# simonsysu/tfs

Measured on AMD Instinct MI355X. Metric: GiB/s CRC32 verify, device-resident 64 KiB files; 1/2/4/8 MI355X, higher is better.
Workload: dtype u8

## Files before the change

### tfs_amd/csrc/tfs_crc_abi.cpp

```cpp
#include <emmintrin.h>
#include <hip/hip_runtime.h>

#include <algorithm>
#include <atomic>
#include <chrono>
#include <condition_variable>
#include <cstdarg>
#include <cstdio>
#include <cstdlib>
#include <cstring>
#include <map>
#include <memory>
#include <mutex>
#include <shared_mutex>
#include <string>
#include <vector>

#include "../../include/tfs_crc.h"
#include "../../include/tfs_crc_testing.h"
#include "../../include/tfs_read.h"
#include "../../include/tfs_receive.h"
#include "../../include/tfs_replicate.h"
#include "../../include/tfs_write.h"
#include "crc_math.h"
#include "pin_registry.h"
#include "mirror_plan.h"
#include "read_reply_plan.h"
#include "receive_plan.h"
#include "replicate_plan.h"
#include "tfs_crc_device.h"

namespace tfscrc {
hipError_t launch_crc_files(int mode, const uint8_t* base, const Desc* desc, uint32_t n, const Tables* tg,
                            uint32_t* out_crc, uint8_t* out_ok, uint32_t* n_bad, uint32_t* sched, hipStream_t stream,
                            int variant, uint32_t vseed, uint32_t* done_flag, uint32_t seq, unsigned cap,
                            const SplitArgs* split);
hipError_t launch_packet_parse(const uint8_t* base, const PacketDesc* pd, uint32_t n, int mode, Desc* desc,
                               int32_t* pre, hipStream_t stream);
hipError_t launch_packet_files(uint8_t* base, const PacketDesc* pd, uint32_t n, int mode, const Tables* tg,
                               uint32_t* crc, int32_t* status, uint32_t* n_bad, uint32_t* sched, hipStream_t stream,
                               unsigned cap);
hipError_t launch_packet_finish(uint8_t* base, const PacketDesc* pd, const Desc* desc, uint32_t n, int mode,
                                const int32_t* pre, const uint8_t* ok, uint32_t* crc, int32_t* status,
                                uint32_t* n_bad, hipStream_t stream);
hipError_t launch_packet_write(const uint8_t* base, const PacketDesc* pd, uint32_t n, const Tables* tg, uint32_t* crc,
                               int32_t* status, uint32_t* n_bad, WritePart* parts, uint32_t* sched,
                               hipStream_t stream, unsigned cap);
hipError_t launch_packet_write_parse(const uint8_t* base, const PacketDesc* pd, uint32_t n, Desc* desc, int32_t* pre,
                                     Desc* hdesc, WritePart* parts, hipStream_t stream);
hipError_t launch_packet_data_fold(const Tables* tg, uint32_t n, const int32_t* status, const uint32_t* crc,
                                   const uint32_t* pcrc, WritePart* parts, hipStream_t stream);
hipError_t launch_crc_shift(const Tables* tg, const uint32_t* crc, const uint32_t* nbytes, uint32_t n, uint32_t* out,
                            hipStream_t stream);
hipError_t launch_block_verify_pipe(const uint8_t* image, uint64_t image_len, const RawMeta* metas,
                                    const CompactJob* jobs, uint32_t n, const Tables* tg, uint32_t* out_crc,
                                    int32_t* out_status, uint32_t* n_bad, uint32_t* sched, hipStream_t stream,
                                    int variant, unsigned cap);
hipError_t launch_compact_fused(const uint8_t* src, uint64_t src_len, const RawMeta* metas, const int32_t* flags,
                                const int64_t* dest_off, uint32_t n, uint8_t* dst, const Tables* tg, uint32_t* out_crc,
                                int32_t* out_status, uint32_t* n_bad, uint32_t* sched, hipStream_t stream,
                                int variant, unsigned cap);
hipError_t launch_compact_jobs(const uint8_t* src, uint64_t src_len, const CompactJob* jobs, uint32_t n, uint8_t* dst,
                               const Tables* tg, uint32_t* out_crc, int32_t* out_status, uint32_t* n_bad,
                               uint32_t* sched, hipStream_t stream, int variant, unsigned cap, const CSegArgs* seg);
hipError_t launch_read_reply(const uint8_t* src, uint64_t src_len, const ReadUnit* units, uint32_t n, uint8_t* out,
                             const Tables* tg, ReadResult* results, uint32_t* n_bad, uint32_t* sched,
                             hipStream_t stream, unsigned cap);
hipError_t launch_replicate(const uint8_t* src, uint64_t src_len, const RepUnit* units, uint32_t nu,
                            const RepFrame* frames, uint32_t nf, uint8_t* out, const Tables* tg, uint32_t* ucrc,
                            uint8_t* cap_bytes, uint32_t* racc, uint32_t* fcrc, uint32_t* sched, hipStream_t stream,
                            unsigned cap);
hipError_t launch_replicate_finish(const RepRec* recs, uint32_t n, const uint8_t* cap_bytes, const uint32_t* racc,
                                   uint32_t* out_crc, int32_t* out_status, hipStream_t stream);
hipError_t launch_receive(const uint8_t* src, const RecvFrame* frames, uint32_t nf, uint32_t nu, uint8_t* image,
                          const Tables* tg, uint32_t* ucrc, uint32_t block_id, uint32_t* words, tfs_receive_part* parts,
                          uint32_t* n_bad, uint32_t* sched, hipStream_t stream, unsigned cap);
hipError_t launch_receive_finish(const RecvRec* recs, uint32_t n, const uint8_t* image, const uint32_t* words,
                                 uint32_t* out_crc, int32_t* out_status, hipStream_t stream);
hipError_t launch_mirror(const uint8_t* src, uint64_t src_len, const MirJob* jobs, uint32_t nj, const MirFrame* frames,
                         uint32_t nf, const MirUnit* units, uint32_t nu, const uint8_t* prefix, uint8_t* out,
                         const Tables* tg, uint32_t* ucrc, uint8_t* cap_bytes, int32_t* jstat, MirResult* results,
                         uint32_t* n_bad, uint32_t* sched, hipStream_t stream, unsigned cap);
hipError_t launch_synth_fill(uint64_t* dst, uint64_t nwords, uint64_t seed, uint64_t first_word, hipStream_t stream);
hipError_t launch_write_headers(uint8_t* image, const uint64_t* rec_off, const uint32_t* len, const uint32_t* crc,
                                uint64_t first_id, uint32_t n, hipStream_t stream);
hipError_t launch_write_packet_headers(uint8_t* base, const uint64_t* rec_off, const uint32_t* len, uint32_t n,
                                       int32_t pcode, int32_t version, uint64_t first_id, hipStream_t stream);
#ifdef TFS_CRC_MEASURE
hipError_t set_res_fence(uint32_t v);
hipError_t launch_membench(int pattern, const uint8_t* base, const Desc* desc, uint32_t n, uint64_t nbytes,
                           uint32_t* out, unsigned grid, hipStream_t stream);
#endif
hipError_t launch_resident(const Tables* tg, const ResHost* hs, uint32_t* left, uint32_t* dstate, unsigned grid,
                           uint32_t idle_ticks,
                           uint32_t life_ticks, uint32_t gen, hipStream_t stream, uint64_t* trace);
}

namespace tfscrc {

namespace {
struct PinRange {
  uintptr_t end;
  uintptr_t dev;
};
std::shared_mutex g_pin_mu;
std::map<uintptr_t, PinRange> g_pins;
}

void pin_register(void* host, size_t bytes, void* dev) {
  if (!host || !dev) return;
  const uintptr_t h = reinterpret_cast<uintptr_t>(host);
  std::unique_lock<std::shared_mutex> g(g_pin_mu);
  g_pins[h] = PinRange{h + (bytes ? bytes : 1), reinterpret_cast<uintptr_t>(dev)};
}

void pin_unregister(void* host) {
  if (!host) return;
  std::unique_lock<std::shared_mutex> g(g_pin_mu);
  g_pins.erase(reinterpret_cast<uintptr_t>(host));
}

bool pin_lookup(const void* p, void** dev) {
  const uintptr_t a = reinterpret_cast<uintptr_t>(p);
  std::shared_lock<std::shared_mutex> g(g_pin_mu);
  auto it = g_pins.upper_bound(a);
  if (it == g_pins.begin()) return false;
  --it;
  if (a >= it->second.end) return false;
  if (dev) *dev = reinterpret_cast<void*>(it->second.dev + (a - it->first));
  return true;
}

}

static_assert(sizeof(tfs_crc_desc) == 16 && sizeof(tfs_crc_vdesc) == 16, "descriptor ABI");
static_assert(sizeof(tfs_raw_meta) == sizeof(tfscrc::RawMeta), "RawMeta ABI");
static_assert(sizeof(tfs_file_info) == 36, "FileInfo ABI");
static_assert(sizeof(tfs_crc_stats) == 64, "stats ABI");
static_assert(sizeof(tfs_packet_desc) == sizeof(tfscrc::PacketDesc), "packet descriptor ABI");
static_assert(sizeof(tfs_write_part) == sizeof(tfscrc::WritePart) && sizeof(tfs_write_part) == 16, "write part ABI");
static_assert(sizeof(tfs_compact_job) == sizeof(tfscrc::CompactJob) && sizeof(tfs_compact_job) == 40, "compact job ABI");
static_assert(sizeof(tfs_read_job) == 48 && sizeof(tfs_read_result) == 16, "read reply ABI");
static_assert(sizeof(tfs_replicate_cfg) == 32, "replicate cfg ABI");
static_assert(sizeof(tfs_receive_cfg) == 16 && sizeof(tfs_receive_desc) == 24 && sizeof(tfs_receive_part) == 16,
              "receive ABI");
static_assert(sizeof(tfs_mirror_cfg) == 16 && sizeof(tfs_mirror_job) == 64 && sizeof(tfs_mirror_result) == 16,
              "mirror ABI");

namespace {

using namespace tfscrc;

struct DevBuf {
  void* p = nullptr;
  size_t cap = 0;
  hipError_t reserve(size_t bytes) {
    if (bytes <= cap) return hipSuccess;
    if (p) (void)hipFree(p);
    p = nullptr;
    cap = 0;
    size_t want = std::max<size_t>(bytes, 4096);
// ... 2782 lines not shown
  if (n == 0) return TFS_SUCCESS;
  HIP_TRY(ctx, hipSetDevice(ctx->device));
  hipStream_t st = ctx->stream;
  const size_t pbytes = size_t(n) * sizeof(tfs_receive_part);
  HIP_TRY(ctx, s->d_parts.reserve(pbytes + 4u));
  HIP_TRY(ctx, s->h_parts.reserve(pbytes + 4u));
  tfs_receive_part* d_parts = static_cast<tfs_receive_part*>(s->d_parts.p);
  uint32_t* d_bad = reinterpret_cast<uint32_t*>(static_cast<uint8_t*>(s->d_parts.p) + pbytes);
  HIP_TRY(ctx, hipMemsetAsync(d_bad, 0, 4u, st));
  void* zbase = nullptr;
  const bool zc = is_pinned_host(base) && host_dev_ptr(base, &zbase);
  (void)hipGetLastError();
  if (zc) {
    if (const int rc = recv_enqueue(s, st, static_cast<const uint8_t*>(zbase), descs, n, d_parts, d_bad)) return rc;
  } else {
    const uint64_t piece = std::max<uint64_t>(ctx->read_piece.load(std::memory_order_relaxed), 1u);
    const uint8_t* b8 = static_cast<const uint8_t*>(base);
    std::vector<tfs_receive_desc> pd;
    for (uint32_t j0 = 0; j0 < n;) {
      uint64_t lo = UINT64_MAX, hi = 0;
      uint32_t j1 = j0;
      pd.clear();
      for (; j1 < n; ++j1) {
        tfs_receive_desc d = descs[j1];
        d.avail = kRecvOverhead + uint32_t(d.data_len);
        const uint64_t nlo = std::min(lo, d.frame_off), nhi = std::max(hi, d.frame_off + d.avail);
        if (j1 > j0 && nhi - nlo > piece) break;
        lo = nlo, hi = nhi;
        pd.push_back(d);
      }
      const uint64_t span = hi - lo, sa = lo & 15u;
      HIP_TRY(ctx, s->h_stage.reserve(span + 32u));
      HIP_TRY(ctx, s->d_stage.reserve(span + 32u));
      memcpy(static_cast<uint8_t*>(s->h_stage.p) + sa, b8 + lo, span);
      HIP_TRY(ctx, hipMemcpyAsync(static_cast<uint8_t*>(s->d_stage.p) + sa, static_cast<uint8_t*>(s->h_stage.p) + sa, span,
                                  hipMemcpyHostToDevice, st));
      for (auto& d : pd) d.frame_off -= lo;
      if (const int rc = recv_enqueue(s, st, static_cast<const uint8_t*>(s->d_stage.p) + sa, pd.data(), j1 - j0,
                                      d_parts + j0, d_bad))
        return rc;
      HIP_TRY(ctx, hipStreamSynchronize(st));
      j0 = j1;
    }
  }
  HIP_TRY(ctx, hipMemcpyAsync(s->h_parts.p, s->d_parts.p, pbytes + 4u, hipMemcpyDeviceToHost, st));
  HIP_TRY(ctx, hipStreamSynchronize(st));
  memcpy(parts, s->h_parts.p, pbytes);
  if (n_bad) {
    uint32_t bad = 0;
    memcpy(&bad, static_cast<const uint8_t*>(s->h_parts.p) + pbytes, 4u);
    *n_bad += bad;
  }
  s->stream = st, s->stream_set = true;
  s->cursor = end;
  return TFS_SUCCESS;
}

int tfs_receive_finish(tfs_receive* s, const tfs_raw_meta* metas, uint32_t n, uint32_t* out_crc, int32_t* out_status,
                       uint32_t* n_bad, int32_t* out_total) {
  if (!s) return TFS_EXIT_PARAMETER_ERROR;
  tfs_crc_ctx* ctx = s->ctx;
  if (s->finished) return set_err(ctx, TFS_EXIT_PARAMETER_ERROR, "receive finish: called twice");
  if (n && !metas) return set_err(ctx, TFS_EXIT_PARAMETER_ERROR, "receive finish: %u records and no metas", n);
  HIP_TRY(ctx, hipSetDevice(ctx->device));
  s->finished = true;
  hipStream_t st = s->stream_set ? s->stream : ctx->stream;
  if (!s->waited) {
    if (st != ctx->stream) HIP_TRY(ctx, hipStreamWaitEvent(st, s->ready, 0));
    s->waited = true;
  }
  const uint32_t* hr = nullptr;
  if (n) {
    s->recs.resize(n);
    s->res.resize(size_t(n) * 2u);
    for (uint32_t i = 0; i < n; ++i) s->recs[i] = recv_make_rec(metas[i], s->cursor);
    const size_t rbytes = size_t(n) * sizeof(RecvRec);
    uint8_t* d_fin = s->fin();
    if (n > kRecvFinRecs) {
      HIP_TRY(ctx, s->d_fin.reserve(rbytes + size_t(n) * 8u));
      d_fin = static_cast<uint8_t*>(s->d_fin.p);
    }
    uint32_t* d_crc = reinterpret_cast<uint32_t*>(d_fin + rbytes);
    HIP_TRY(ctx, hipMemcpyAsync(d_fin, s->recs.data(), rbytes, hipMemcpyHostToDevice, st));
    HIP_TRY(ctx, launch_receive_finish(reinterpret_cast<const RecvRec*>(d_fin), n, s->d_image, s->words(), d_crc,
                                       reinterpret_cast<int32_t*>(d_crc + n), st));
    HIP_TRY(ctx, hipMemcpyAsync(s->res.data(), d_crc, size_t(n) * 8u, hipMemcpyDeviceToHost, st));
    hr = s->res.data();
  }
  HIP_TRY(ctx, hipStreamSynchronize(st));
  uint32_t bad = 0;
  for (uint32_t i = 0; i < n; ++i) {
    const int32_t status = int32_t(hr[n + i]);
    if (out_crc) out_crc[i] = hr[i];
    if (out_status) out_status[i] = status;
    bad += status != TFS_SUCCESS ? 1u : 0u;
  }
  if (n_bad) *n_bad += bad;
  if (out_total) *out_total = int32_t(s->cursor);
  return TFS_SUCCESS;
}

int tfs_receive_free(tfs_receive* s) {
  if (!s) return TFS_EXIT_PARAMETER_ERROR;
  (void)hipSetDevice(s->ctx->device);
  if (s->stream_set) (void)hipStreamSynchronize(s->stream);
  if (!s->waited && s->ready) (void)hipEventSynchronize(s->ready);
  s->release();
  delete s;
  return TFS_SUCCESS;
}


extern "C++" {
namespace {

int mir_call_checks(tfs_crc_ctx* ctx, const tfs_mirror_cfg* cfg, const void* src, uint64_t src_len,
                    const tfs_mirror_job* jobs, uint32_t n, const uint64_t* ds, uint32_t ds_n, const void* out,
                    uint64_t out_cap, const void* results, std::vector<int32_t>* pre) {
  if (!cfg || !out || !results || (n && !jobs) || (ds_n && !ds) || (src_len && !src)) return TFS_EXIT_PARAMETER_ERROR;
  if (!mir_cfg_ok(*cfg))
    return set_err(ctx, TFS_EXIT_PARAMETER_ERROR, "mirror: first_len %d, frame_len %d, reserved %d are refused",
                   cfg->first_len, cfg->frame_len, int(cfg->reserved));
  pre->resize(n);
  for (uint32_t i = 0; i < n; ++i) (*pre)[i] = mir_pre_status(*cfg, jobs[i], ds_n, src_len, out_cap);
  if (mir_spans_overlap(*cfg, jobs, pre->data(), n))
    return set_err(ctx, TFS_EXIT_PARAMETER_ERROR, "mirror: the spans of two jobs overlap");
  return TFS_SUCCESS;
}

int mir_enqueue(tfs_crc_ctx* ctx, hipStream_t st, const uint8_t* d_src, uint64_t src_len, const tfs_mirror_cfg& cfg,
                const tfs_mirror_job* jobs, const int32_t* pre, uint32_t n, const uint64_t* ds, uint8_t* d_out,
                tfs_mirror_result* d_results, uint32_t* d_n_bad) {
  std::lock_guard<std::mutex> g(ctx->mir_mu);
  MirPlan& p = ctx->mir_plan;
  if (!make_mirror_plan(cfg, jobs, pre, n, ds, &p))
    return set_err(ctx, TFS_EXIT_PARAMETER_ERROR, "mirror: more than 2^31 frames or units in one call");
  const uint32_t nf = uint32_t(p.frames.size()), nu = uint32_t(p.units.size());
  const size_t o_frames = up16(size_t(n) * sizeof(MirJob)), o_units = o_frames + size_t(nf) * sizeof(MirFrame);
  const size_t o_prefix = o_units + size_t(nu) * sizeof(MirUnit), plan_bytes = up16(o_prefix + p.prefix.size());
  const size_t o_ucrc = plan_bytes, o_cap = o_ucrc + up16(size_t(nu) * 4u);
  const size_t o_jstat = o_cap + up16(size_t(n) * kFileInfoSize), total = o_jstat + size_t(n) * 4u;
  ReadPlanSlot& rp = ctx->mir_plans[ctx->mir_plan_next++ % kReadPlanRing];
  if (rp.done) HIP_TRY(ctx, hipEventSynchronize(rp.done));
  HIP_TRY(ctx, rp.h.reserve(plan_bytes));
  HIP_TRY(ctx, rp.d.reserve(total));
  uint8_t* h8 = static_cast<uint8_t*>(rp.h.p);
  uint8_t* d8 = static_cast<uint8_t*>(rp.d.p);
  memcpy(h8, p.jobs.data(), size_t(n) * sizeof(MirJob));
  if (nf) memcpy(h8 + o_frames, p.frames.data(), size_t(nf) * sizeof(MirFrame));
  if (nu) memcpy(h8 + o_units, p.units.data(), size_t(nu) * sizeof(MirUnit));
  if (!p.prefix.empty()) memcpy(h8 + o_prefix, p.prefix.data(), p.prefix.size());
  HIP_TRY(ctx, hipMemcpyAsync(d8, h8, plan_bytes, hipMemcpyHostToDevice, st));
  SCHED_LAUNCH(ctx, st, "mirror",
               launch_mirror(d_src, src_len, reinterpret_cast<const MirJob*>(d8), n,
                             reinterpret_cast<const MirFrame*>(d8 + o_frames), nf,
                             reinterpret_cast<const MirUnit*>(d8 + o_units), nu, d8 + o_prefix, d_out, ctx->d_tables,
                             reinterpret_cast<uint32_t*>(d8 + o_ucrc), d8 + o_cap,
                             reinterpret_cast<int32_t*>(d8 + o_jstat), d_results, d_n_bad, sched, st,
                             throughput_cap(ctx)));
  if (!rp.done) HIP_TRY(ctx, hipEventCreateWithFlags(&rp.done, hipEventDisableTiming));
  HIP_TRY(ctx, hipEventRecord(rp.done, st));
  return TFS_SUCCESS;
}

}
}

// ... 538 lines not shown
```

### tfs_amd/csrc/tfs_crc_kernels.hip

```cpp
#include <hip/hip_runtime.h>
#include <stdint.h>

#include <type_traits>

#include "mirror_plan.h"
#include "read_reply_plan.h"
#include "receive_plan.h"
#include "replicate_plan.h"
#include "tfs_crc_device.h"

namespace tfscrc {

typedef const __attribute__((address_space(1))) uint32_t* gu32p;
typedef unsigned int u32x4 __attribute__((ext_vector_type(4)));
typedef const __attribute__((address_space(1))) u32x4* gu128p;
typedef const __attribute__((address_space(1))) uint8_t* gu8p;
__device__ __forceinline__ uint32_t ld32(uintptr_t a) { return *reinterpret_cast<gu32p>(a); }
__device__ __forceinline__ uint4 ld128(uintptr_t a) {
  const u32x4 v = *reinterpret_cast<gu128p>(a);
  return make_uint4(v.x, v.y, v.z, v.w);
}
template <bool NT>
__device__ __forceinline__ uint4 ld128s(uintptr_t a) {
  if (NT) {
// ... 2046 lines not shown
  const uint32_t g = off / kRecvG + (f - u0);
  const uint64_t gs = uint64_t(g) * kRecvG, fe = uint64_t(off) + len;
  const uint64_t start = gs > off ? gs : uint64_t(off);
  const uint64_t end = gs + kRecvG < fe ? gs + kRecvG : fe;
  RepUnit u{};
  u.soff = soff + kRecvHead + (start - off);
  u.doff = start;
  u.plen = uint32_t(end - start);
  src_end = recv_uni(frames[lo].src_end);
  return u;
}

__global__ void __launch_bounds__(kBlock, 4) receive_kernel(const uint8_t* __restrict__ src,
                                                            const RecvFrame* __restrict__ frames_in, uint32_t nf,
                                                            uint32_t n, uint8_t* __restrict__ image,
                                                            const Tables* __restrict__ tg, uint32_t* __restrict__ ucrc,
                                                            uint32_t* sched) {
  __shared__ uint32_t lds_tables[LdsLayout<kLY>::bytes / 4];
  __shared__ uint32_t lds_frames[kRecvLdsFrames * sizeof(RecvFrame) / 4];
  if (nf <= kRecvLdsFrames) {
    const uint32_t* f32 = reinterpret_cast<const uint32_t*>(frames_in);
    for (uint32_t k = threadIdx.x; k < nf * uint32_t(sizeof(RecvFrame) / 4); k += kBlock) lds_frames[k] = f32[k];
  }
  load_tables<kRun, kPAR, kLY>(lds_tables, tg);
  __syncthreads();
  const RecvFrame* frames = nf <= kRecvLdsFrames ? reinterpret_cast<const RecvFrame*>(lds_frames) : frames_in;
  const int lane = threadIdx.x & (kWave - 1);
  const LaneBase lb = lane_base_for<kLY>(lane);
  const uint32_t wpb = kBlock / kWave;
  const uintptr_t junk = reinterpret_cast<uintptr_t>(tg->slice);
  FileCursor<kIL, 1, 0, kCompactHS> fc;
  fc.init(sched, n, blockIdx.x & 7u, gridDim.x * wpb,
          blockIdx.x * wpb + __builtin_amdgcn_readfirstlane(threadIdx.x / kWave));
  fc.start(lane);
  do {
    uint32_t f = __builtin_amdgcn_readfirstlane(fc.take(lane));
    if (f >= n) break;
    uint32_t fn = __builtin_amdgcn_readfirstlane(fc.take(lane));
    uint64_t cur_end = 0, nxt_end = 0;
    RepUnit cur = recv_unit(frames, nf, f, cur_end);
    CState st = issue_rep(cur, src, cur_end, image, lane, junk);
    uint4 buf[kPF][kRun / 16];
    load_ring<kRun, kPF, false>(st.g, lane, buf, junk);
    RepUnit nxt = fn < n ? recv_unit(frames, nf, fn, nxt_end) : RepUnit{};
    for (;;) {
      const bool more = fn < n;
      const RepUnit ncur = nxt;
      uint32_t c = st.g.nstripes ? lane_chain<kRun, kPF, false, kLY, true, true, 1>(lds_tables, lb, st.g, st.h, buf,
                                                                                    lane, junk, st.delta, true)
                                 : 0u;
      CState ns = st;
      uint32_t fnn = n;
      if (more) {
        ns = issue_rep(ncur, src, nxt_end, image, lane, junk);
        load_ring<kRun, kPF, false>(ns.g, lane, buf, junk);
        fnn = __builtin_amdgcn_readfirstlane(fc.take(lane));
        if (fnn < n) nxt = recv_unit(frames, nf, fnn, nxt_end);
      }
      if (st.g.nstripes) {
        if (lane == 0) {
          const uint32_t ntw = uint32_t((st.g.end & ~uintptr_t(3)) - st.g.B16) / 4u;
          for (uint32_t i = 0; i < 3u; ++i)
            if (i < ntw) st32u(st.g.B16 + 4u * i + st.delta, st.h.tw[i]);
          const uintptr_t B = st.g.end & ~uintptr_t(3);
          for (uint32_t i = 0; i < 3u; ++i)
            if (B + i < st.g.end) *reinterpret_cast<uint8_t*>(B + i + st.delta) = uint8_t(st.h.tb[i]);
        }
      } else {
        copy_unaligned(src + cur.soff, image + cur.doff, cur.plen, lane);
      }
      c = finish_file<kRun, kLY>(lds_tables, lb, st.g, st.h, c, lane);
      if (lane == 0) ucrc[f] = c;
      if (!more) break;
      f = fn;
      fn = fnn;
      cur = ncur;
      st = ns;
    }
  } while (false);
  if (lane == 0) launch_exit(sched, gridDim.x * wpb, nullptr, 0u);
}

__device__ const RecvPowTab kRecvPow = recv_pow_tab();
__device__ __forceinline__ uint32_t recv_pow(uint32_t d) {
  uint32_t r = 0x80000000u;
  for (uint32_t k = 0; d; ++k, d >>= 1)
    if (d & 1u) r = gf_mul(r, kRecvPow.p[k]);
  return r;
}

__device__ __forceinline__ uint32_t recv_byte_crc(uint32_t b) {
#pragma unroll
  for (int k = 0; k < 8; ++k) b = (b >> 1) ^ ((b & 1u) ? kPoly : 0u);
  return b;
}

__device__ __forceinline__ uint32_t recv_wave_xor(uint32_t x) {
#pragma unroll
  for (int m = kWave / 2; m >= 1; m >>= 1) x ^= __shfl_xor(x, m, kWave);
  return x;
}

__device__ __forceinline__ uint32_t recv_dword(uint32_t hb, uint32_t k) {
  return __shfl(hb, int(4u * k), kWave) | __shfl(hb, int(4u * k + 1u), kWave) << 8 |
         __shfl(hb, int(4u * k + 2u), kWave) << 16 | __shfl(hb, int(4u * k + 3u), kWave) << 24;
}

__global__ void __launch_bounds__(kWave) receive_fold_kernel(const uint8_t* __restrict__ src,
                                                             const RecvFrame* __restrict__ frames,
                                                             const uint32_t* __restrict__ ucrc, uint32_t block_id,
                                                             uint32_t* words, tfs_receive_part* __restrict__ parts,
                                                             uint32_t* n_bad) {
  const RecvFrame fr = frames[blockIdx.x];
  const uint32_t lane = threadIdx.x;
  const uint8_t* frame = src + fr.soff;
  uint32_t hb = 0u;
  if (lane < kRecvHead) hb = frame[lane];
  else if (lane < kRecvOverhead) hb = frame[uint64_t(fr.len) + lane];
  const uint32_t h_flag = recv_dword(hb, 0), h_body = recv_dword(hb, 1), h_tv = recv_dword(hb, 2);
  const uint32_t h_crc = recv_dword(hb, 5), i_block = recv_dword(hb, 6), i_off = recv_dword(hb, 9);
  const uint32_t i_len = recv_dword(hb, 10), flag = recv_dword(hb, 14);
  const bool in_h = lane >= 24u && lane < kRecvHead, in_f = lane >= kRecvHead && lane < kRecvOverhead;
  const uint32_t bc = (in_h || in_f) ? gf_mul(recv_byte_crc(hb), recv_pow(in_h ? 55u - lane : 59u - lane)) : 0u;
  const uint32_t ch = recv_wave_xor(in_h ? bc : 0u), cf = recv_wave_xor(in_f ? bc : 0u);
  uint32_t x = 0u;
  const uint32_t g0 = fr.off / kRecvG, fe = fr.off + fr.len;
  const uint32_t nb = fr.nu ? fr.nu - 1u : 0u;
  const uint32_t per = (nb + kWave - 1u) / kWave;
  const uint32_t k0 = lane * per, k1 = k0 + per < nb ? k0 + per : nb;
  uint32_t acc = 0u;
  for (uint32_t k = k0; k < k1; ++k) {
    const uint32_t c = ucrc[fr.u0 + k];
    acc = gf_mul(acc, kRecvPow.p[kRecvLgG]) ^ c;
    if ((g0 + k) * kRecvG >= fr.off) words[g0 + k] = c;
    else atomicXor(&words[g0 + k], c);
  }
  if (k0 < k1) x = gf_mul(acc, recv_pow(fe - (g0 + k1) * kRecvG));
  if (lane == kWave - 1 && fr.nu) {
    const uint32_t c = ucrc[fr.u0 + nb];
    const uint32_t gs = (g0 + nb) * kRecvG;
    x ^= c;
    if (gs >= fr.off && fe == gs + kRecvG) words[g0 + nb] = c;
    else atomicXor(&words[g0 + nb], gf_mul(c, recv_pow(gs + kRecvG - fe)));
  }
  x = recv_wave_xor(x);
  if (lane == 0) {
    const uint32_t chs = ch ^ gf_mul(kPacketFlagV1, kRecvPow.p[5]);
    const uint32_t body = gf_mul(chs, recv_pow(fr.len + 4u)) ^ gf_mul(x, kRecvPow.p[2]) ^ cf;
    const int32_t version = int16_t(uint16_t(h_tv >> 16));
    int32_t status = kSuccess;
    if (h_flag != kPacketFlagV1) status = TFS_ERROR;
    else if (h_body != kRecvInfo + fr.len) status = TFS_ERROR;
    else if ((h_tv & 0xffffu) != uint32_t(TFS_RECEIVE_PCODE)) status = TFS_ERROR;
    else if (i_block != block_id) status = TFS_ERROR;
    else if (i_off != fr.off || i_len != fr.len) status = TFS_ERROR;
    else if (version >= 1 && h_crc != body) status = kExitCheckCrcError;
    parts[blockIdx.x] = tfs_receive_part{status, version >= 1 ? body : 0u, int32_t(flag), 0u};
    if (status != kSuccess && n_bad) atomicAdd(n_bad, 1u);
  }
}

__device__ __forceinline__ uint32_t recv_edge(const uint8_t* __restrict__ image, uint32_t lo, uint32_t hi, uint32_t b,
                                              uint32_t lane) {
  constexpr uint32_t kPer = kRecvG / kWave;
  if (hi - lo <= lane * kPer) return 0u;
  const uint32_t e = hi - lane * kPer;
  const uint32_t s = e - lo > kPer ? e - kPer : lo;
  uint32_t c = 0u;
  for (uint32_t i = s; i < e; ++i) {
    c ^= image[i];
#pragma unroll
    for (int k = 0; k < 8; ++k) c = (c >> 1) ^ ((c & 1u) ? kPoly : 0u);
  }
  return gf_mul(c, recv_pow(b - e));
}

__global__ void __launch_bounds__(kWave) receive_finish_kernel(const RecvRec* __restrict__ recs, uint32_t n,
                                                                const uint8_t* __restrict__ image,
                                                                const uint32_t* __restrict__ words,
                                                                uint32_t* __restrict__ out_crc,
                                                                int32_t* __restrict__ out_status) {
  const uint32_t i = blockIdx.x;
  if (i >= n) return;
  const uint32_t lane = threadIdx.x;
  const RecvRec r = recs[i];
  if (r.pre != kSuccess) {
    if (lane == 0) out_crc[i] = 0u, out_status[i] = r.pre;
    return;
  }
  const uint32_t hb = lane < kRecvInfo ? uint32_t(image[uint64_t(uint32_t(r.offset)) + lane]) : 0u;
  const uint64_t id = uint64_t(recv_dword(hb, 0)) | uint64_t(recv_dword(hb, 1)) << 32;
  const uint32_t fi_size = recv_dword(hb, 3), fi_crc = recv_dword(hb, 8);
  uint32_t x = recv_edge(image, r.a, r.he, r.b, lane) ^ recv_edge(image, r.tb, r.b, r.b, lane);
  if (lane < r.ng) {
    const uint32_t mstep = kRecvPow.p[kRecvLgG + 6u];
    uint32_t acc = 0u, first = 0u;
    for (uint32_t k = lane % kWave; k < r.ng; k += kWave) first = k;
    for (uint32_t k = first;; k -= kWave) {
      acc = gf_mul(acc, mstep) ^ words[r.g0 + r.ng - 1u - k];
      if (k < kWave) break;
    }
    x ^= gf_mul(acc, recv_pow(r.b - (r.g0 + r.ng - lane) * kRecvG));
  }
  x = recv_wave_xor(x);
  if (lane == 0) {
    int32_t status = kSuccess;
    if (id != r.file_id) status = kExitFileInfoError;
    else if (int32_t(fi_size) != r.size) status = kExitSyncFileError;
    else if (x != fi_crc) status = kExitCheckCrcError;
    out_crc[i] = x;
    out_status[i] = status;
  }
}

__device__ __forceinline__ CState issue_mir(const MirUnit& u, const uint8_t* src, uint64_t src_len, uint8_t* out,
                                            int lane, uintptr_t junk) {
  CRec r;
  r.soff = u.soff - kFileInfoSize;
  r.doff = u.doff - kFileInfoSize;
  r.fid = 0;
  r.size = 0, r.flag = 0, r.new_off = 0;
  r.pre = kSuccess;
  r.plen = u.plen;
  r.kind = 1u;
  r.edge = 0u;
  CState s = issue_crec<true>(r, src, src_len, out, lane, junk);
  s.hb = (u.job & kMirStart) && lane < kFileInfoSize ? uint32_t(src[r.soff + uint32_t(lane)]) : 0u;
  return s;
}

__global__ void __launch_bounds__(kBlock, 4) mirror_kernel(const uint8_t* __restrict__ src, uint64_t src_len,
                                                           const MirUnit* __restrict__ units, uint32_t n,
                                                           uint8_t* __restrict__ out, const Tables* __restrict__ tg,
                                                           uint32_t* __restrict__ ucrc, uint8_t* __restrict__ cap,
                                                           uint32_t* sched) {
  __shared__ uint32_t lds_tables[LdsLayout<kLY>::bytes / 4];
  load_tables<kRun, kPAR, kLY>(lds_tables, tg);
  const int lane = threadIdx.x & (kWave - 1);
  const LaneBase lb = lane_base_for<kLY>(lane);
  const uint32_t wpb = kBlock / kWave;
  const uintptr_t junk = reinterpret_cast<uintptr_t>(tg->slice);
  FileCursor<kIL, 1, 0, kCompactHS> fc;
  fc.init(sched, n, blockIdx.x & 7u, gridDim.x * wpb,
          blockIdx.x * wpb + __builtin_amdgcn_readfirstlane(threadIdx.x / kWave));
  fc.start(lane);
  do {
    uint32_t f = fc.take(lane);
    if (f >= n) break;
    uint32_t fn = fc.take(lane);
    MirUnit cur = units[f];
    CState st = issue_mir(cur, src, src_len, out, lane, junk);
    uint4 buf[kPF][kRun / 16];
    load_ring<kRun, kPF, false>(st.g, lane, buf, junk);
    MirUnit nxt = fn < n ? units[fn] : MirUnit{};
    for (;;) {
      const bool more = fn < n;
      const MirUnit ncur = nxt;
      uint32_t c = st.g.nstripes ? lane_chain<kRun, kPF, false, kLY, true, true, 1>(lds_tables, lb, st.g, st.h, buf,
                                                                                    lane, junk, st.delta, true)
                                 : 0u;
      CState ns = st;
      uint32_t fnn = n;
      if (more) {
        ns = issue_mir(ncur, src, src_len, out, lane, junk);
        load_ring<kRun, kPF, false>(ns.g, lane, buf, junk);
        fnn = fc.take(lane);
        if (fnn < n) nxt = units[fnn];
      }
      if ((cur.job & kMirStart) && lane < kFileInfoSize)
        cap[uint64_t(cur.job & ~kMirStart) * kFileInfoSize + uint32_t(lane)] = uint8_t(st.hb);
      if (st.g.nstripes) {
        if (lane == 0) {
          const uint32_t ntw = uint32_t((st.g.end & ~uintptr_t(3)) - st.g.B16) / 4u;
          for (uint32_t i = 0; i < 3u; ++i)
            if (i < ntw) st32u(st.g.B16 + 4u * i + st.delta, st.h.tw[i]);
          const uintptr_t B = st.g.end & ~uintptr_t(3);
          for (uint32_t i = 0; i < 3u; ++i)
            if (B + i < st.g.end) *reinterpret_cast<uint8_t*>(B + i + st.delta) = uint8_t(st.h.tb[i]);
        }
      } else {
        copy_unaligned(src + cur.soff, out + cur.doff, cur.plen, lane);
      }
      c = finish_file<kRun, kLY>(lds_tables, lb, st.g, st.h, c, lane);
      if (lane == 0) ucrc[f] = c;
      if (!more) break;
// ... 729 lines not shown
  else if (variant == 96) TFS_CJ(12, 2, 2, 3, kCompactDiag);
  else if (variant == 97) TFS_CJ(16, 1, 2, kPF, kCompactDiag);
  else if (variant == 98) TFS_CJ(10, 2, 2, kPF, kCompactDiag);
  else if (variant == 99) TFS_CJ(16, 2, 2, 3, kCompactDiag);
  else if (variant == 120) TFS_CJR(16, 1, 2, kPF, kCompactDiag, true);
  else if (variant == 121) TFS_CJR(8, 1, 2, 8, kCompactDiag, true);
  else
#endif
    TFS_CJ(16, 1, kLY, kPF, kCompactDiag);
#undef TFS_CJ
#undef TFS_CJR
  (void)variant;
  return hipGetLastError();
}

hipError_t launch_block_verify_pipe(const uint8_t* image, uint64_t image_len, const RawMeta* metas,
                                    const CompactJob* jobs, uint32_t n, const Tables* tg, uint32_t* out_crc,
                                    int32_t* out_status, uint32_t* n_bad, uint32_t* sched, hipStream_t stream,
                                    int variant, unsigned cap) {
  if (n == 0) return hipSuccess;
  if (!sched) return hipErrorInvalidValue;
  const dim3 grid(grid_for(n, cap));
#define TFS_BV(WIDE_, CF_, TS_)                                                                                     \
  hipLaunchKernelGGL((compact_pipe_kernel<WIDE_, true, kCompactDiag, kPF, CF_, TS_>), grid, dim3(kBlock), 0, stream, \
                     image, image_len, metas, nullptr, nullptr, jobs, n, nullptr, tg, out_crc, out_status, n_bad, sched, \
                     CSegArgs{nullptr, 0u, 0u})
#ifdef TFS_CRC_MEASURE
  if (variant == 50 && jobs) TFS_BV(true, 1, 0);
  else if (variant == 50) TFS_BV(false, 1, 0);
  else
#endif
  if (jobs) TFS_BV(true, kCF, kTS);
  else TFS_BV(false, kCF, kTS);
#undef TFS_BV
  (void)variant;
  return hipGetLastError();
}

hipError_t launch_read_reply(const uint8_t* src, uint64_t src_len, const ReadUnit* units, uint32_t n, uint8_t* out,
                             const Tables* tg, ReadResult* results, uint32_t* n_bad, uint32_t* sched,
                             hipStream_t stream, unsigned cap) {
  if (n == 0) return hipSuccess;
  if (!sched) return hipErrorInvalidValue;
  hipLaunchKernelGGL(read_reply_kernel, dim3(grid_for(n, cap)), dim3(kBlock), 0, stream, src, src_len, units, n, out,
                     tg, results, n_bad, sched);
  return hipGetLastError();
}

hipError_t launch_replicate(const uint8_t* src, uint64_t src_len, const RepUnit* units, uint32_t nu,
                            const RepFrame* frames, uint32_t nf, uint8_t* out, const Tables* tg, uint32_t* ucrc,
                            uint8_t* cap_bytes, uint32_t* racc, uint32_t* fcrc, uint32_t* sched, hipStream_t stream,
                            unsigned cap) {
  if (nf == 0) return hipSuccess;
  if (nu) {
    if (!sched) return hipErrorInvalidValue;
    hipLaunchKernelGGL(replicate_kernel, dim3(grid_for(nu, cap)), dim3(kBlock), 0, stream, src, src_len, units, nu, out,
                       tg, ucrc, cap_bytes, sched);
    const hipError_t e = hipGetLastError();
    if (e != hipSuccess) return e;
  }
  hipLaunchKernelGGL(replicate_fold_kernel, dim3(nf), dim3(kWave), 0, stream, frames, units, ucrc, out, racc, fcrc);
  return hipGetLastError();
}

hipError_t launch_replicate_finish(const RepRec* recs, uint32_t n, const uint8_t* cap_bytes, const uint32_t* racc,
                                   uint32_t* out_crc, int32_t* out_status, hipStream_t stream) {
  if (n == 0) return hipSuccess;
  hipLaunchKernelGGL(replicate_finish_kernel, dim3((n + 255u) / 256u), dim3(256), 0, stream, recs, n, cap_bytes, racc,
                     out_crc, out_status);
  return hipGetLastError();
}

hipError_t launch_receive(const uint8_t* src, const RecvFrame* frames, uint32_t nf, uint32_t nu, uint8_t* image,
                          const Tables* tg, uint32_t* ucrc, uint32_t block_id, uint32_t* words, tfs_receive_part* parts,
                          uint32_t* n_bad, uint32_t* sched, hipStream_t stream, unsigned cap) {
  if (nf == 0) return hipSuccess;
  if (nu) {
    if (!sched) return hipErrorInvalidValue;
    hipLaunchKernelGGL(receive_kernel, dim3(grid_for(nu, cap)), dim3(kBlock), 0, stream, src, frames, nf, nu, image, tg,
                       ucrc, sched);
    const hipError_t e = hipGetLastError();
    if (e != hipSuccess) return e;
  }
  hipLaunchKernelGGL(receive_fold_kernel, dim3(nf), dim3(kWave), 0, stream, src, frames, ucrc, block_id, words, parts,
                     n_bad);
  return hipGetLastError();
}

hipError_t launch_receive_finish(const RecvRec* recs, uint32_t n, const uint8_t* image, const uint32_t* words,
                                 uint32_t* out_crc, int32_t* out_status, hipStream_t stream) {
  if (n == 0) return hipSuccess;
  hipLaunchKernelGGL(receive_finish_kernel, dim3(n), dim3(kWave), 0, stream, recs, n, image, words,
                     out_crc, out_status);
  return hipGetLastError();
}

hipError_t launch_mirror(const uint8_t* src, uint64_t src_len, const MirJob* jobs, uint32_t nj, const MirFrame* frames,
                         uint32_t nf, const MirUnit* units, uint32_t nu, const uint8_t* prefix, uint8_t* out,
                         const Tables* tg, uint32_t* ucrc, uint8_t* cap_bytes, int32_t* jstat, MirResult* results,
                         uint32_t* n_bad, uint32_t* sched, hipStream_t stream, unsigned cap) {
  if (nj == 0) return hipSuccess;
  if (nu) {
    if (!sched) return hipErrorInvalidValue;
    hipLaunchKernelGGL(mirror_kernel, dim3(grid_for(nu, cap)), dim3(kBlock), 0, stream, src, src_len, units, nu, out, tg,
                       ucrc, cap_bytes, sched);
    const hipError_t e = hipGetLastError();
    if (e != hipSuccess) return e;
  }
  hipLaunchKernelGGL(mirror_job_fold_kernel, dim3(nj), dim3(kWave), 0, stream, jobs, units, ucrc, cap_bytes, results,
                     jstat, n_bad);
  const hipError_t e = hipGetLastError();
  if (e != hipSuccess || nf == 0) return e;
  hipLaunchKernelGGL(mirror_frame_fold_kernel, dim3(nf), dim3(kWave), 0, stream, frames, jobs, units, ucrc, prefix, jstat,
                     out);
  return hipGetLastError();
}

hipError_t launch_synth_fill(uint64_t* dst, uint64_t nwords, uint64_t seed, uint64_t first_word, hipStream_t stream) {
  if (nwords == 0) return hipSuccess;
  uint64_t g = (nwords + 255) / 256;
  if (g > 65536) g = 65536;
  hipLaunchKernelGGL(synth_fill_kernel, dim3(unsigned(g)), dim3(256), 0, stream, dst, nwords, seed, first_word);
  return hipGetLastError();
}

#ifdef TFS_CRC_MEASURE
template <int PF, int SK, int HOLE = 0>
__global__ void __launch_bounds__(kBlock) membench_copy_chunk_kernel(const uint8_t* __restrict__ src,
                                                                     uint8_t* __restrict__ dst, uint64_t nbytes,
                                                                     uint64_t ch) {
  const int lane = threadIdx.x & (kWave - 1);
  const uint64_t wave = uint64_t(blockIdx.x) * (kBlock / kWave) + __builtin_amdgcn_readfirstlane(threadIdx.x / kWave);
  const uint64_t nw = uint64_t(gridDim.x) * (kBlock / kWave);
  const uint64_t nch = nbytes / ch;
  const uintptr_t s = reinterpret_cast<uintptr_t>(src), d = reinterpret_cast<uintptr_t>(dst);
  for (uint64_t c = wave; c < nch; c += nw) {
    const uint64_t b = c * ch + 16u * uint64_t(lane);
    for (uint64_t o = 0; o < ch; o += 1024u * PF) {
      uint4 v[PF];
#pragma unroll
      for (int k = 0; k < PF; ++k) v[k] = ld128s<true>(s + b + o + 1024u * k);
#pragma unroll
      for (int k = 0; k < PF; ++k) {
        const u32x4 w = {v[k].x, v[k].y, v[k].z, v[k].w};
        gu128wp a = reinterpret_cast<gu128wp>(d + b + o + 1024u * k);
        const bool first = o == 0 && k == 0 && lane == 0;
        const bool last = o + 1024u * (k + 1) >= ch && k == PF - 1 && lane == kWave - 1;
        if (HOLE && (first || (HOLE >= 2 && last))) {
          if (HOLE == 3) {
            uint8_t* bp = reinterpret_cast<uint8_t*>(d + b + o + 1024u * k);
            const uint32_t ww[4] = {w[0], w[1], w[2], w[3]};
#pragma unroll
            for (int i = 0; i < 16; ++i) bp[i] = uint8_t(ww[i >> 2] >> (8 * (i & 3)));
          }
          continue;
        }
        if (SK == 1) __builtin_nontemporal_store(w, a);
        else *a = w;
      }
    }
  }
}




hipError_t launch_membench(int pattern, const uint8_t* base, const Desc* desc, uint32_t n, uint64_t nbytes,
                           uint32_t* out, unsigned grid, hipStream_t stream) {
  if (pattern >= 53000 && pattern < 54000) {
    const int S = (pattern / 100) % 10, CC = pattern % 100;
    const uint64_t ch = uint64_t(CC ? CC : 4) * 16384u;
    const uint64_t nb = nbytes / ch * ch;
    const dim3 g(grid ? grid : kMaxGrid);
    uint8_t* d = reinterpret_cast<uint8_t*>(out);
    if (S == 1)
      hipLaunchKernelGGL((membench_copy_chunk_kernel<8, 1>), g, dim3(kBlock), 0, stream, base, d, nb, ch);
// ... 55 lines not shown
```

Before: 6201.

## Use LDS shift and slice tables in receive fold and finish kernels

After: 6135. 0.989x the previous value.

```diff
diff --git a/tfs_amd/csrc/tfs_crc_abi.cpp b/tfs_amd/csrc/tfs_crc_abi.cpp
--- a/tfs_amd/csrc/tfs_crc_abi.cpp
+++ b/tfs_amd/csrc/tfs_crc_abi.cpp
@@ -76,7 +76,7 @@
                           const Tables* tg, uint32_t* ucrc, uint32_t block_id, uint32_t* words, tfs_receive_part* parts,
                           uint32_t* n_bad, uint32_t* sched, hipStream_t stream, unsigned cap);
 hipError_t launch_receive_finish(const RecvRec* recs, uint32_t n, const uint8_t* image, const uint32_t* words,
-                                 uint32_t* out_crc, int32_t* out_status, hipStream_t stream);
+                                 const Tables* tg, uint32_t* out_crc, int32_t* out_status, hipStream_t stream);
 hipError_t launch_mirror(const uint8_t* src, uint64_t src_len, const MirJob* jobs, uint32_t nj, const MirFrame* frames,
                          uint32_t nf, const MirUnit* units, uint32_t nu, const uint8_t* prefix, uint8_t* out,
                          const Tables* tg, uint32_t* ucrc, uint8_t* cap_bytes, int32_t* jstat, MirResult* results,
@@ -3025,7 +3025,8 @@
     }
     uint32_t* d_crc = reinterpret_cast<uint32_t*>(d_fin + rbytes);
     HIP_TRY(ctx, hipMemcpyAsync(d_fin, s->recs.data(), rbytes, hipMemcpyHostToDevice, st));
-    HIP_TRY(ctx, launch_receive_finish(reinterpret_cast<const RecvRec*>(d_fin), n, s->d_image, s->words(), d_crc,
+    HIP_TRY(ctx, launch_receive_finish(reinterpret_cast<const RecvRec*>(d_fin), n, s->d_image, s->words(), ctx->d_tables,
+                                       d_crc,
                                        reinterpret_cast<int32_t*>(d_crc + n), st));
     HIP_TRY(ctx, hipMemcpyAsync(s->res.data(), d_crc, size_t(n) * 8u, hipMemcpyDeviceToHost, st));
     hr = s->res.data();
diff --git a/tfs_amd/csrc/tfs_crc_kernels.hip b/tfs_amd/csrc/tfs_crc_kernels.hip
--- a/tfs_amd/csrc/tfs_crc_kernels.hip
+++ b/tfs_amd/csrc/tfs_crc_kernels.hip
@@ -2152,18 +2152,39 @@
 }
 
 __device__ const RecvPowTab kRecvPow = recv_pow_tab();
-__device__ __forceinline__ uint32_t recv_pow(uint32_t d) {
-  uint32_t r = 0x80000000u;
-  for (uint32_t k = 0; d; ++k, d >>= 1)
-    if (d & 1u) r = gf_mul(r, kRecvPow.p[k]);
-  return r;
-}
-
-__device__ __forceinline__ uint32_t recv_byte_crc(uint32_t b) {
-#pragma unroll
-  for (int k = 0; k < 8; ++k) b = (b >> 1) ^ ((b & 1u) ? kPoly : 0u);
-  return b;
-}
+
+constexpr uint32_t kRecvLvlDw = uint32_t(kAnyLevels) * kAnyStride / 4u;
+constexpr uint32_t kRecvSliceOff = kRecvLvlDw * 4u;
+static_assert(offsetof(Tables, any_shift) % 16 == 0 && kRecvLvlDw % 4u == 0, "the tables are staged 16 bytes a load");
+static_assert(kRecvLgG + 6u < uint32_t(kAnyLevels), "a step of 64 granules is one level");
+template <uint32_t NS>
+__device__ __forceinline__ void recv_load_tables(uint32_t* L, const Tables* __restrict__ tg) {
+  uint4* l4 = reinterpret_cast<uint4*>(L);
+  const uint4* a4 = reinterpret_cast<const uint4*>(&tg->any_shift[0][0][0]);
+  const uint4* s4 = reinterpret_cast<const uint4*>(&tg->slice[0][0]);
+  for (uint32_t k = threadIdx.x; k < kRecvLvlDw / 4u; k += blockDim.x) l4[k] = a4[k];
+  for (uint32_t k = threadIdx.x; k < NS * 64u; k += blockDim.x) l4[kRecvLvlDw / 4u + k] = s4[k];
+  __syncthreads();
+}
+
+__device__ __forceinline__ uint32_t recv_shift(const uint32_t* L, uint32_t c, uint32_t d) {
+  uint32_t lo = d & ((1u << kAnyLevels) - 1u);
+#pragma unroll 1
+  for (uint32_t off = 0u; lo; lo >>= 1, off += kAnyStride)
+    if (lo & 1u) c = shift5(L, off, c);
+#pragma unroll 1
+  for (uint32_t k = uint32_t(kAnyLevels), hi = d >> kAnyLevels; hi; ++k, hi >>= 1)
+    if (hi & 1u) c = gf_mul(c, kRecvPow.p[k]);
+  return c;
+}
+__device__ __forceinline__ uint32_t recv_level(const uint32_t* L, uint32_t k, uint32_t c) {
+  return shift5(L, k * kAnyStride, c);
+}
+
+__device__ __forceinline__ uint32_t recv_byte_crc(const uint32_t* L, uint32_t b) {
+  return lds_ld(L, kRecvSliceOff + (b << 2));
+}
+constexpr uint32_t kRecvFlagShift32 = recv_cmul(kPacketFlagV1, recv_pow_tab().p[5]);
 
 __device__ __forceinline__ uint32_t recv_wave_xor(uint32_t x) {
 #pragma unroll
@@ -2176,13 +2197,17 @@
          __shfl(hb, int(4u * k + 2u), kWave) << 16 | __shfl(hb, int(4u * k + 3u), kWave) << 24;
 }
 
-__global__ void __launch_bounds__(kWave) receive_fold_kernel(const uint8_t* __restrict__ src,
-                                                             const RecvFrame* __restrict__ frames,
-                                                             const uint32_t* __restrict__ ucrc, uint32_t block_id,
-                                                             uint32_t* words, tfs_receive_part* __restrict__ parts,
-                                                             uint32_t* n_bad) {
-  const RecvFrame fr = frames[blockIdx.x];
-  const uint32_t lane = threadIdx.x;
+constexpr uint32_t kRecvFoldWaves = 8;
+__global__ void __launch_bounds__(kRecvFoldWaves * kWave)
+    receive_fold_kernel(const uint8_t* __restrict__ src, const RecvFrame* __restrict__ frames, uint32_t nf,
+                        const uint32_t* __restrict__ ucrc, uint32_t block_id, const Tables* __restrict__ tg,
+                        uint32_t* words, tfs_receive_part* __restrict__ parts, uint32_t* n_bad) {
+  __shared__ __attribute__((aligned(16))) uint32_t L[kRecvLvlDw + 256u];
+  recv_load_tables<1>(L, tg);
+  const uint32_t fi = blockIdx.x * kRecvFoldWaves + recv_uni(uint32_t(threadIdx.x) / kWave);
+  if (fi >= nf) return;
+  const RecvFrame fr = frames[fi];
+  const uint32_t lane = threadIdx.x & (kWave - 1);
   const uint8_t* frame = src + fr.soff;
   uint32_t hb = 0u;
   if (lane < kRecvHead) hb = frame[lane];
@@ -2191,8 +2216,10 @@
   const uint32_t h_crc = recv_dword(hb, 5), i_block = recv_dword(hb, 6), i_off = recv_dword(hb, 9);
   const uint32_t i_len = recv_dword(hb, 10), flag = recv_dword(hb, 14);
   const bool in_h = lane >= 24u && lane < kRecvHead, in_f = lane >= kRecvHead && lane < kRecvOverhead;
-  const uint32_t bc = (in_h || in_f) ? gf_mul(recv_byte_crc(hb), recv_pow(in_h ? 55u - lane : 59u - lane)) : 0u;
+  const uint32_t bc =
+      (in_h || in_f) ? recv_shift(L, recv_byte_crc(L, hb), in_h ? kRecvHead - 1u - lane : kRecvOverhead - 1u - lane) : 0u;
   const uint32_t ch = recv_wave_xor(in_h ? bc : 0u), cf = recv_wave_xor(in_f ? bc : 0u);
+  const uint32_t hs = recv_shift(L, ch ^ kRecvFlagShift32, fr.len + 4u);
   uint32_t x = 0u;
   const uint32_t g0 = fr.off / kRecvG, fe = fr.off + fr.len;
   const uint32_t nb = fr.nu ? fr.nu - 1u : 0u;
@@ -2201,22 +2228,21 @@
   uint32_t acc = 0u;
   for (uint32_t k = k0; k < k1; ++k) {
     const uint32_t c = ucrc[fr.u0 + k];
-    acc = gf_mul(acc, kRecvPow.p[kRecvLgG]) ^ c;
+    acc = recv_level(L, kRecvLgG, acc) ^ c;
     if ((g0 + k) * kRecvG >= fr.off) words[g0 + k] = c;
     else atomicXor(&words[g0 + k], c);
   }
-  if (k0 < k1) x = gf_mul(acc, recv_pow(fe - (g0 + k1) * kRecvG));
+  if (k0 < k1) x = recv_shift(L, acc, fe - (g0 + k1) * kRecvG);
   if (lane == kWave - 1 && fr.nu) {
     const uint32_t c = ucrc[fr.u0 + nb];
     const uint32_t gs = (g0 + nb) * kRecvG;
     x ^= c;
     if (gs >= fr.off && fe == gs + kRecvG) words[g0 + nb] = c;
-    else atomicXor(&words[g0 + nb], gf_mul(c, recv_pow(gs + kRecvG - fe)));
+    else atomicXor(&words[g0 + nb], recv_shift(L, c, gs + kRecvG - fe));
   }
   x = recv_wave_xor(x);
   if (lane == 0) {
-    const uint32_t chs = ch ^ gf_mul(kPacketFlagV1, kRecvPow.p[5]);
-    const uint32_t body = gf_mul(chs, recv_pow(fr.len + 4u)) ^ gf_mul(x, kRecvPow.p[2]) ^ cf;
+    const uint32_t body = hs ^ recv_level(L, 2u, x) ^ cf;
     const int32_t version = int16_t(uint16_t(h_tv >> 16));
     int32_t status = kSuccess;
     if (h_flag != kPacketFlagV1) status = TFS_ERROR;
@@ -2225,34 +2251,43 @@
     else if (i_block != block_id) status = TFS_ERROR;
     else if (i_off != fr.off || i_len != fr.len) status = TFS_ERROR;
     else if (version >= 1 && h_crc != body) status = kExitCheckCrcError;
-    parts[blockIdx.x] = tfs_receive_part{status, version >= 1 ? body : 0u, int32_t(flag), 0u};
+    parts[fi] = tfs_receive_part{status, version >= 1 ? body : 0u, int32_t(flag), 0u};
     if (status != kSuccess && n_bad) atomicAdd(n_bad, 1u);
   }
 }
 
-__device__ __forceinline__ uint32_t recv_edge(const uint8_t* __restrict__ image, uint32_t lo, uint32_t hi, uint32_t b,
-                                              uint32_t lane) {
+__device__ __forceinline__ uint32_t recv_edge(const uint32_t* L, const uint8_t* __restrict__ image, uint32_t lo,
+                                              uint32_t hi, uint32_t b, uint32_t lane) {
   constexpr uint32_t kPer = kRecvG / kWave;
   if (hi - lo <= lane * kPer) return 0u;
   const uint32_t e = hi - lane * kPer;
   const uint32_t s = e - lo > kPer ? e - kPer : lo;
-  uint32_t c = 0u;
-  for (uint32_t i = s; i < e; ++i) {
-    c ^= image[i];
-#pragma unroll
-    for (int k = 0; k < 8; ++k) c = (c >> 1) ^ ((c & 1u) ? kPoly : 0u);
-  }
-  return gf_mul(c, recv_pow(b - e));
-}
-
-__global__ void __launch_bounds__(kWave) receive_finish_kernel(const RecvRec* __restrict__ recs, uint32_t n,
-                                                                const uint8_t* __restrict__ image,
-                                                                const uint32_t* __restrict__ words,
-                                                                uint32_t* __restrict__ out_crc,
-                                                                int32_t* __restrict__ out_status) {
-  const uint32_t i = blockIdx.x;
+  const uint8_t* p = image + s;
+  uint32_t left = e - s, c = 0u;
+  for (; left && (reinterpret_cast<uintptr_t>(p) & 3u); ++p, --left) c = (c >> 8) ^ recv_byte_crc(L, (c ^ *p) & 0xffu);
+  for (; left >= 4u; p += 4, left -= 4u) {
+    const uint32_t v = c ^ *reinterpret_cast<const uint32_t*>(p);
+    c = xor3(lds_ld(L, kRecvSliceOff + 3072u + ((v << 2) & 0x3FCu)), lds_ld(L, kRecvSliceOff + 2048u + ((v >> 6) & 0x3FCu)),
+             lds_ld(L, kRecvSliceOff + 1024u + ((v >> 14) & 0x3FCu))) ^
+        lds_ld(L, kRecvSliceOff + ((v >> 22) & 0x3FCu));
+  }
+  for (; left; ++p, --left) c = (c >> 8) ^ recv_byte_crc(L, (c ^ *p) & 0xffu);
+  return recv_shift(L, c, b - e);
+}
+
+#ifndef TFS_RECV_FIN_WAVES
+#define TFS_RECV_FIN_WAVES 4
+#endif
+constexpr uint32_t kRecvFinWaves = TFS_RECV_FIN_WAVES;
+__global__ void __launch_bounds__(kRecvFinWaves * kWave)
+    receive_finish_kernel(const RecvRec* __restrict__ recs, uint32_t n, const uint8_t* __restrict__ image,
+                          const uint32_t* __restrict__ words, const Tables* __restrict__ tg,
+                          uint32_t* __restrict__ out_crc, int32_t* __restrict__ out_status) {
+  __shared__ __attribute__((aligned(16))) uint32_t L[kRecvLvlDw + 1024u];
+  recv_load_tables<4>(L, tg);
+  const uint32_t i = blockIdx.x * kRecvFinWaves + recv_uni(uint32_t(threadIdx.x) / kWave);
   if (i >= n) return;
-  const uint32_t lane = threadIdx.x;
+  const uint32_t lane = threadIdx.x & (kWave - 1);
   const RecvRec r = recs[i];
   if (r.pre != kSuccess) {
     if (lane == 0) out_crc[i] = 0u, out_status[i] = r.pre;
@@ -2261,16 +2296,15 @@
   const uint32_t hb = lane < kRecvInfo ? uint32_t(image[uint64_t(uint32_t(r.offset)) + lane]) : 0u;
   const uint64_t id = uint64_t(recv_dword(hb, 0)) | uint64_t(recv_dword(hb, 1)) << 32;
   const uint32_t fi_size = recv_dword(hb, 3), fi_crc = recv_dword(hb, 8);
-  uint32_t x = recv_edge(image, r.a, r.he, r.b, lane) ^ recv_edge(image, r.tb, r.b, r.b, lane);
+  uint32_t x = recv_edge(L, image, r.a, r.he, r.b, lane) ^ recv_edge(L, image, r.tb, r.b, r.b, lane);
   if (lane < r.ng) {
-    const uint32_t mstep = kRecvPow.p[kRecvLgG + 6u];
     uint32_t acc = 0u, first = 0u;
     for (uint32_t k = lane % kWave; k < r.ng; k += kWave) first = k;
     for (uint32_t k = first;; k -= kWave) {
-      acc = gf_mul(acc, mstep) ^ words[r.g0 + r.ng - 1u - k];
+      acc = recv_level(L, kRecvLgG + 6u, acc) ^ words[r.g0 + r.ng - 1u - k];
       if (k < kWave) break;
     }
-    x ^= gf_mul(acc, recv_pow(r.b - (r.g0 + r.ng - lane) * kRecvG));
+    x ^= recv_shift(L, acc, r.b - (r.g0 + r.ng - lane) * kRecvG);
   }
   x = recv_wave_xor(x);
   if (lane == 0) {
@@ -3166,16 +3200,16 @@
     const hipError_t e = hipGetLastError();
     if (e != hipSuccess) return e;
   }
-  hipLaunchKernelGGL(receive_fold_kernel, dim3(nf), dim3(kWave), 0, stream, src, frames, ucrc, block_id, words, parts,
-                     n_bad);
+  hipLaunchKernelGGL(receive_fold_kernel, dim3((nf + kRecvFoldWaves - 1u) / kRecvFoldWaves),
+                     dim3(kRecvFoldWaves * kWave), 0, stream, src, frames, nf, ucrc, block_id, tg, words, parts, n_bad);
   return hipGetLastError();
 }
 
 hipError_t launch_receive_finish(const RecvRec* recs, uint32_t n, const uint8_t* image, const uint32_t* words,
-                                 uint32_t* out_crc, int32_t* out_status, hipStream_t stream) {
+                                 const Tables* tg, uint32_t* out_crc, int32_t* out_status, hipStream_t stream) {
   if (n == 0) return hipSuccess;
-  hipLaunchKernelGGL(receive_finish_kernel, dim3(n), dim3(kWave), 0, stream, recs, n, image, words,
-                     out_crc, out_status);
+  hipLaunchKernelGGL(receive_finish_kernel, dim3((n + kRecvFinWaves - 1u) / kRecvFinWaves), dim3(kRecvFinWaves * kWave),
+                     0, stream, recs, n, image, words, tg, out_crc, out_status);
   return hipGetLastError();
 }
 
```
